# SheepYang666/VINA-SLAM

Measured on AMD Instinct MI355X. Metric: scans/sec (downsample+kNN+LM solve), 64-line LiDAR, 1/2/4/8 MI355X; ATE vs CPU, higher is better.
Workload: dtype f64

## Files before the change

### vina-slam_amd/csrc/insert.hip

```cpp
#include <cstring>
#include <vector>
#include "vg_map.h"

namespace vg {

template <bool kPre>
__global__ void __launch_bounds__(256) k_ins_prep(int n_arg, const int* __restrict__ nd, const float* __restrict__ ox, const float* __restrict__ oy,
                           const float* __restrict__ oz, const float* __restrict__ oi, MP mp, DState* __restrict__ st, int slot,
                           DevMap m, double* __restrict__ pw, uint32_t* __restrict__ hslot,
                           const PushArg* __restrict__ pa, const double* __restrict__ pin, const double* __restrict__ xsrc,
                           int var_identity, int* __restrict__ dsf, unsigned long long* __restrict__ gran, int ngran,
                           const int* __restrict__ ph_in) {
  const int n = nd ? *nd : n_arg;
  {
    const int g = blockIdx.x * blockDim.x + threadIdx.x;
    if (gran && g < ngran) gran[g] = 0ull;
  }
  if (!kPre && pa && blockIdx.x == 0) push_state_block(st, *pa);
  if (ph_in && blockIdx.x == 0 && threadIdx.x < 6) st->ph[threadIdx.x] = ph_in[threadIdx.x];
  const double* xc = kPre ? xsrc : st->xc;
  M3 R, rot_var, tsl_var;
  for (int r = 0; r < 3; r++)
    for (int c = 0; c < 3; c++) {
      R(r, c) = xc[r * 3 + c];
// ... 216 lines not shown
    const int upto = last ? ntile : b;
    int a0 = 0, a1 = 0, a2 = 0, t0 = 0, t1 = 0, t2 = 0;
    for (int k = lane; k < upto; k += 64) {
      u64 g;
      for (long it = 0;; it++) {
        g = __hip_atomic_load(&gran[k], __ATOMIC_RELAXED, __HIP_MEMORY_SCOPE_AGENT);
        if (g >> 63) break;
        __builtin_amdgcn_s_sleep(1);
        if (it > (1l << 24)) {
          atomicOr(&m.counters[kCntErr], 64);
          g = 1ull << 63;
          break;
        }
      }
      const int c0 = (int)(g & kF), c1 = (int)((g >> 21) & kF), c2 = (int)((g >> 42) & kF);
      if (k < b) {
        a0 += c0;
        a1 += c1;
        a2 += c2;
      }
      t0 += c0;
      t1 += c1;
      t2 += c2;
    }
    for (int o = 32; o > 0; o >>= 1) {
      a0 += __shfl_down(a0, o, 64);
      a1 += __shfl_down(a1, o, 64);
      a2 += __shfl_down(a2, o, 64);
      t0 += __shfl_down(t0, o, 64);
      t1 += __shfl_down(t1, o, 64);
      t2 += __shfl_down(t2, o, 64);
    }
    if (lane == 0) {
      s_off[0] = a0;
      s_off[1] = a1;
      s_off[2] = a2;
      s_tot[0] = t0;
      s_tot[1] = t1;
      s_tot[2] = t2;
    }
  }
  __syncthreads();
  const int base = m.counters[kCntNew], sbase = m.counters[kCntSlideBase];
#pragma unroll
  for (int k = 0; k < 4; k++) {
    const int i = i0 + k;
    const int cd = code[k];
    const u64 rk = r;
    r += pack3(cd);
    if (i >= n || !(cd & 1)) continue;
    const uint32_t s = hslot[i];
    int rt;
    if (cd & 2) {
      rt = base + s_off[1] + (int)((rk >> 21) & kF);
      if (rt >= m.cap_nodes) {
        atomicOr(&m.counters[kCntErr], 4);
        continue;
      }
      const uint64_t key = m.hkey[s];
      double c[3];
      const int64_t kk[3] = {unpack_axis(key, 42), unpack_axis(key, 21), unpack_axis(key, 0)};
      for (int j = 0; j < 3; j++) c[j] = (0.5 + kk[j]) * mp.vs;
      init_node(m.hdr[rt], c, (float)(mp.vs / 4.0), 0, -1);
      dbox_root(m.dbox + (size_t)rt * 6);
      m.hval[s] = rt;
    } else {
      rt = m.hval[s];
      m.hdr[rt].isexist = 1;
    }
    if (cd & 4) {
      m.in_slide[rt] = 1;
      m.slide[sbase + s_off[2] + (int)((rk >> 42) & kF)] = rt;
    }
    m.hfirst[s] = 0x7f7f7f7f;
  }
  if (b == ntile - 1 && tid == 0) {
    m.counters[kCntNodes] = min(base + s_tot[1], m.cap_nodes);
    m.counters[kCntRoots] = s_tot[1];
    m.counters[kCntTouched] = s_tot[0];
    m.counters[kCntSlide] = sbase + s_tot[2];
  }
}

__device__ __forceinline__ bool ins_skip(const DevMap& m, int thread_num) {
  return g_touched(m) < thread_num || m.counters[kCntMisc] != 0;
}

template <bool kCount>
__global__ void __launch_bounds__(256) k_ins_descend(int n_arg, const int* __restrict__ nd, int thread_num, const double* __restrict__ pw, DevMap m,
                                                     const uint32_t* __restrict__ hslot, int* __restrict__ leaf,
                                                     int* __restrict__ reqlist, int* __restrict__ seg_key) {
  const int n = nd ? *nd : n_arg;
  if (ins_skip(m, thread_num)) return;
  for (int base = blockIdx.x * blockDim.x; base < n; base += gridDim.x * blockDim.x) {
    const int i = base + threadIdx.x;
    int node = -1;
    bool first = false;
    if (i < n) {
      const uint32_t hs = hslot[i];
      node = hs != 0xffffffffu ? m.hval[hs] : -1;
    }
    if (node >= 0) {
      V3 w = v3(pw[3 * i], pw[3 * i + 1], pw[3 * i + 2]);
      for (int d = 0; d < 8; d++) {
        const NodeHdr& h = m.hdr[node];
        if (h.octo == 0) break;
        int o = octant(w, h.center);
        int c = h.child[o];
        if (c < 0) {
          if (atomicCAS(&m.cfirst[(size_t)node * 8 + o], 0x7f7f7f7f, -5) == 0x7f7f7f7f) {
            first = true;
            if (atomicExch(&m.nscr[(size_t)node * 4 + 1], -7) != -7) {
              int pos = atomicAdd(&m.counters[kCntCreate], 1);
              reqlist[pos] = node;
            }
          }
          if (kCount) atomicAdd(&m.creq_cnt[(size_t)node * 8 + o], 1);
          node = -2 - (node * 8 + o);
          break;
        }
        node = c;
      }
      if (kCount && node >= 0) first = atomicAdd(&m.leaf_cnt[node], 1) == 0;
    }
    if (i < n) leaf[i] = node;
    if (kCount) {
      const int s = wave_append(&m.counters[kCntSeg], first ? 1 : 0);
      if (first) seg_key[s] = node;
    }
  }
}

__global__ void __launch_bounds__(256) k_ins_resolve(int n_arg, const int* __restrict__ nd, int thread_num, const double* __restrict__ pw, DevMap m,
                                                     int* __restrict__ leaf, int* __restrict__ seg_leaf) {
  const int n = nd ? *nd : n_arg;
  if (ins_skip(m, thread_num)) return;
  for (int base = blockIdx.x * blockDim.x; base < n; base += gridDim.x * blockDim.x) {
    const int i = base + threadIdx.x;
    int node = i < n ? leaf[i] : -1;
    if (node < -1) {
      const int code = -2 - node;
      node = m.hdr[code >> 3].child[code & 7];
      leaf[i] = node;
    }
    const bool first = node >= 0 && atomicAdd(&m.leaf_cnt[node], 1) == 0;
    const int s = wave_append(&m.counters[kCntSeg], first ? 1 : 0);
    if (first) {
      seg_leaf[s] = node;
      m.leaf_seg[node] = s;
    }
  }
}

__global__ void __launch_bounds__(1024) k_seg_offsets(int thread_num, DevMap m, const int* __restrict__ seg_leaf,
                                                      int* __restrict__ seg_off) {
  __shared__ int s_w[17];
  if (ins_skip(m, thread_num)) return;
  const int ns = m.counters[kCntSeg];
  const int per = (ns + (int)blockDim.x - 1) / (int)blockDim.x;
  const int s0 = threadIdx.x * per, s1 = min(ns, s0 + per);
  constexpr int kPer = 32;
  int total;
  if (per <= kPer) {
    int lf[kPer], c[kPer];
#pragma unroll
    for (int k = 0; k < kPer; k++) lf[k] = s0 + k < s1 ? seg_leaf[s0 + k] : -1;
    int cnt = 0;
#pragma unroll
    for (int k = 0; k < kPer; k++) {
      c[k] = lf[k] >= 0 ? m.leaf_cnt[lf[k]] : 0;
      cnt += c[k];
    }
    int pos = block_excl_scan(cnt, s_w, &total);
#pragma unroll
    for (int k = 0; k < kPer; k++)
      if (lf[k] >= 0) {
        seg_off[s0 + k] = pos;
        pos += c[k];
        m.leaf_cnt[lf[k]] = 0;
      }
  } else {
    int cnt = 0;
// ... 298 lines not shown
                                                        int cap, const int* __restrict__ seg_key,
                                                        int2* __restrict__ seg_ol) {
  __shared__ int sp[kInsAllocCap];
  __shared__ int s_w[17];
  if (blockIdx.x == 0) {
    ins_alloc_block(thread_num, m, reqlist, cap, sp, s_w);
    return;
  }
  if (g_touched(m) < thread_num) return;
  const int ns = m.counters[kCntSeg];
  for (int base = ((int)blockIdx.x - 1) * (int)blockDim.x; base < ns; base += ((int)gridDim.x - 1) * (int)blockDim.x) {
    const int s = base + threadIdx.x;
    int* c = s < ns ? seg_counter(m, seg_key[s]) : nullptr;
    const int len = c ? *c : 0;
    const int off = wave_append(&m.counters[kCntSegCur], len);
    if (c) {
      seg_ol[s] = make_int2(off, len);
      *c = off;
    }
  }
}

__global__ void __launch_bounds__(256) k_ins_scatter_cur(int n_arg, const int* __restrict__ nd, int thread_num, DevMap m,
                                                         const int* __restrict__ leaf, int* __restrict__ order) {
  const int n = nd ? *nd : n_arg;
  if (ins_skip(m, thread_num)) return;
  for (int i = blockIdx.x * blockDim.x + threadIdx.x; i < n; i += gridDim.x * blockDim.x) {
    const int l = leaf[i];
    if (l == -1) continue;
    order[atomicAdd(seg_counter(m, l), 1)] = i;
  }
}

static int insert_tail(vg_ctx* ctx, const MP& mp, int slot, int n, int thread_num, const int* nd = nullptr) {
  DevMap& m = ctx->map;
  Work& w = ctx->wk;
  hipStream_t s = ctx->stream;
  const int g = grid_for(n);
  const int gseg = (n + kPushWaves - 1) / kPushWaves < 2048 ? (n + kPushWaves - 1) / kPushWaves : 2048;
  int* seg_leaf = w.list1;
  int* seg_off = reinterpret_cast<int*>(w.v0);
  int* order = reinterpret_cast<int*>(w.k0);
  int* order2 = reinterpret_cast<int*>(w.k1);
  const bool cur = ctx->ins_count;
  if (cur) {
    k_ins_scatter_cur<<<g * (kBlock / kSpreadBlock), kSpreadBlock, 0, s>>>(n, nd, thread_num, m, w.leaf, order);
  } else {
    k_ins_resolve<<<g * (kBlock / kSpreadBlock), kSpreadBlock, 0, s>>>(n, nd, thread_num, w.pw, m, w.leaf, seg_leaf);
    k_seg_offsets<<<1, 1024, 0, s>>>(thread_num, m, seg_leaf, seg_off);
    k_ins_scatter<<<g * (kBlock / kSpreadBlock), kSpreadBlock, 0, s>>>(n, nd, thread_num, m, w.leaf, seg_off, order);
  }
  RcBeginArg rb;
  memset(&rb, 0, sizeof(rb));
  const bool has_rb = ctx->rc_begin_wa != nullptr;
  if (has_rb) {
    rb.wa = *ctx->rc_begin_wa;
    rb.st = ctx->st;
    rb.wpn = m.wpn;
    rb.win = (WinD*)ctx->ba.xs;
    rb.nper = (int*)((char*)ctx->ba.xs + sizeof(WinD));
    rb.slot_of = rb.nper + 32;
    rb.rc = w.rc;
    ctx->rc_begin_wa = nullptr;
    ctx->rc_begun = true;
  }
  auto push = cur ? (ctx->push_pipe ? k_push_window<true, true> : k_push_window<true, false>)
                  : (ctx->push_pipe ? k_push_window<false, true> : k_push_window<false, false>);
  push<<<gseg + (has_rb ? 1 : 0), 64 * kPushWaves, 0, s>>>(seg_leaf, seg_off, order, order2, mp, slot, m, w.pw, thread_num,
                                                            rb, has_rb ? 1 : 0);
  VG_HIP(hipGetLastError());
  return VG_OK;
}

int map_insert(vg_ctx* ctx, const MP& mp, int slot, int n, int epoch, int thread_num, const PushArg* push,
               const InsPre* pre, const int* nd) {
  DevMap& m = ctx->map;
  Work& w = ctx->wk;
  hipStream_t s = ctx->stream;
  if (n <= 0) {
    if (push) VG_TRY(state_push(ctx, push->ord, push->new_imu, push->rec));
    return VG_OK;
  }
  const int g = nd ? grid_for(n, kBlock, 2048) : grid_for(n);
  if (pre)
    k_ins_prep<true><<<g, kBlock, 0, s>>>(n, nullptr, nullptr, nullptr, nullptr, nullptr, mp, ctx->st, slot, m, w.pw,
                                          w.u0,
                                          nullptr, pre->pnt, pre->pose, pre->var_identity, nullptr, w.gran, w.ngran,
                                          nullptr);
  else {
    HostIn* hin = ctx->h_in + ctx->in_sel;
    HostIn* din = ctx->d_in + ctx->in_sel;
    if (push) hin->push = *push;
    k_ins_prep<false><<<g, kBlock, 0, s>>>(n, nd, ctx->ds.ox, ctx->ds.oy, ctx->ds.oz, ctx->ds.oi, mp, ctx->st, slot, m,
                                           w.pw,
                                           w.u0, push ? &din->push : nullptr, nullptr, nullptr, 0,
                                           nd ? ctx->ds.hflags : nullptr, w.gran, w.ngran,
                                           ctx->in_ph ? din->ph : nullptr);
  }
  const int ntile = (n + kRootTile - 1) / kRootTile;
  (void)epoch;
  if (ctx->roots_lb && ntile <= w.ngran) {
    k_ins_roots_lb<<<ntile, kBlock, 0, s>>>(n, nd, ntile, w.u0, mp, m, w.gran);
  } else {
    k_ins_flags<<<ntile, kBlock, 0, s>>>(n, nd, w.u0, m, w.v1, (int*)w.ac_cnt);
    k_ins_roots_alloc<<<ntile, kBlock, 0, s>>>(n, nd, ntile, w.u0, w.v1, (const int*)w.ac_cnt, mp, m);
  }
  if (sharded(ctx)) {
    VG_TRY(shard_allreduce(ctx, m.counters + kCntTouched, m.counters + kCntGTouched, 1, 1, 1));
  }
  const int ins_cap = (ctx->dbg_ins_cap >= 0 && ctx->dbg_ins_cap < kInsAllocCap) ? ctx->dbg_ins_cap : kInsAllocCap;
  if (ctx->ins_count) {
    k_ins_descend<true><<<g * (kBlock / kSpreadBlock), kSpreadBlock, 0, s>>>(n, nd, thread_num, w.pw, m, w.u0, w.leaf,
                                                                             w.list2, w.list1);
    k_ins_alloc_seg<<<1 + kSegAllocBlocks, 1024, 0, s>>>(thread_num, m, w.list2, ins_cap, w.list1,
                                                         reinterpret_cast<int2*>(w.v0));
  } else {
    k_ins_descend<false><<<g * (kBlock / kSpreadBlock), kSpreadBlock, 0, s>>>(n, nd, thread_num, w.pw, m, w.u0, w.leaf,
                                                                              w.list2, nullptr);
    k_ins_alloc<<<1, 1024, 0, s>>>(thread_num, m, w.list2, ins_cap);
  }
  return insert_tail(ctx, mp, slot, n, thread_num, nd);
}

int map_insert_replay(vg_ctx* ctx, const MP& mp, int slot, int n, int thread_num) {
  DevMap& m = ctx->map;
  hipStream_t s = ctx->stream;
  VG_TRY(read_counters(ctx));
  const int np = ctx->h_pinned[kCntCreate];
  VG_HIP(hipMemsetAsync(m.counters + kCntMisc, 0, sizeof(int), s));
  if (!ctx->ins_count) VG_HIP(hipMemsetAsync(m.counters + kCntSeg, 0, sizeof(int), s));
  int created = 0;
  VG_TRY(alloc_children(ctx, ctx->wk.list2, np, nullptr, 0, false, &created));
  return insert_tail(ctx, mp, slot, n, thread_num);
}

int map_insert_segments(vg_ctx* ctx, int* key, int* len, int cap, int* info) {
  DevMap& m = ctx->map;
  Work& w = ctx->wk;
  hipStream_t s = ctx->stream;
  int hc[kCntN];
  VG_HIP(hipMemcpyAsync(hc, m.counters, sizeof(hc), hipMemcpyDeviceToHost, s));
  VG_HIP(hipStreamSynchronize(s));
  const int ns = hc[kCntSeg];
  info[0] = ns;
  info[1] = hc[kCntTouched];
  info[2] = hc[kCntCreate];
  info[3] = hc[kCntMisc];
  const int k = ns < cap ? ns : cap;
  if (k <= 0) return VG_OK;
  std::vector<int> off((size_t)2 * k + 2);
  VG_HIP(hipMemcpyAsync(key, w.list1, (size_t)k * sizeof(int), hipMemcpyDeviceToHost, s));
  VG_HIP(hipMemcpyAsync(off.data(), w.v0, (ctx->ins_count ? (size_t)2 * k : (size_t)k + 1) * sizeof(int),
                        hipMemcpyDeviceToHost, s));
  VG_HIP(hipStreamSynchronize(s));
  for (int q = 0; q < k; q++) len[q] = ctx->ins_count ? off[2 * q + 1] : off[q + 1] - off[q];
  return VG_OK;
}

}
```

### vina-slam_amd/csrc/map.hip

```cpp
#include <hipcub/hipcub.hpp>
#include "vg_map.h"

namespace vg {

int map_alloc(vg_ctx* ctx) {
  DevMap& m = ctx->map;
  const int W = ctx->cfg.win_size;
  m.W = W;
  m.cap_nodes = ctx->cap.max_nodes;
  m.cap_fix = ctx->cap.max_fix_points;
  m.hash_mask = (1 << ctx->cap.hash_log2) - 1;
  m.cap_wp = ctx->cap.max_points_per_scan;
  const size_t cn = m.cap_nodes, hs = (size_t)m.hash_mask + 1, cw = (size_t)m.cap_wp;
  auto ok = [&](void* p) { return p != nullptr; };
  bool good = true;
  good &= ok(m.hdr = ctx->arena.take<NodeHdr>(cn));
  good &= ok(m.pl = ctx->arena.take<PlaneRec>(cn));
  good &= ok(m.pcr_add = ctx->arena.take<Clu>(cn));
  good &= ok(m.pcr_fix = ctx->arena.take<Clu>(cn));
  good &= ok(m.cov_add = ctx->arena.take<double>(cn * kCovN));
  good &= ok(m.eig = ctx->arena.take<double>(cn * 12));
  good &= ok(m.jour = ctx->arena.take<double>(cn));
  good &= ok(m.dbox = ctx->arena.take<double>(cn * 6));
  good &= ok(m.pcrs = ctx->arena.take<Clu>(cn * W));
  good &= ok(m.nscr = ctx->arena.take<int>(cn * 4));
  good &= ok(m.pend = ctx->arena.take<unsigned long long>(cn));
  good &= ok(m.cfirst = ctx->arena.take<int>(cn * 8));
  good &= ok(m.hkey = ctx->arena.take<uint64_t>(hs));
  good &= ok(m.hval = ctx->arena.take<int>(hs));
  good &= ok(m.hfirst = ctx->arena.take<int>(hs));
  good &= ok(m.slide = ctx->arena.take<int>(cn));
  good &= ok(m.in_slide = ctx->arena.take<uint8_t>(cn));
  good &= ok(m.leaf_cnt = ctx->arena.take<int>(cn));
  good &= ok(m.leaf_seg = ctx->arena.take<int>(cn));
  good &= ok(m.creq_cnt = ctx->arena.take<int>(cn * 8));
  good &= ok(m.fix_pnt = ctx->arena.take<double>((size_t)m.cap_fix * 3));
  good &= ok(m.fix_var = ctx->arena.take<double>((size_t)m.cap_fix * 9));
  good &= ok(m.wp_pnt = ctx->arena.take<double>(cw * W * 3));
  good &= ok(m.wp_var = ctx->arena.take<double>(cw * W * 9));
  good &= ok(m.wp_leaf = ctx->arena.take<int>(cw * W));
  good &= ok(m.wp_int = ctx->arena.take<float>(cw * W));
  m.ord_stride = (int)(cw * (size_t)(ctx->cfg.max_layer + 1));
  good &= ok(m.wp_ord = ctx->arena.take<int>((size_t)m.ord_stride * W));
  good &= ok(m.lseg = ctx->arena.take<uint64_t>(cn * W));
  good &= ok(m.slot_epoch = ctx->arena.take<int>(kMaxWin));
  good &= ok(m.arena = ctx->arena.take<int>(kMaxWin));
  good &= ok(ctx->d_cmap = ctx->arena.take<float4>((cw + 2) / 3));
  good &= ok(ctx->d_cmap_n = ctx->arena.take<int>(4));
  good &= ok(m.counters = ctx->arena.take<int>(kCntN));
  good &= ok(m.stamp = ctx->arena.take<int>(cn));
  good &= ok(m.wpn = ctx->arena.take<int>(kMaxWin));
  Work& w = ctx->wk;
  w.cap = (int)(cw * (W + 1));
  good &= ok(w.k0 = ctx->arena.take<uint64_t>(w.cap));
  good &= ok(w.k1 = ctx->arena.take<uint64_t>(w.cap));
  good &= ok(w.v0 = ctx->arena.take<uint32_t>(w.cap));
  good &= ok(w.v1 = ctx->arena.take<uint32_t>(w.cap));
  good &= ok(w.u0 = ctx->arena.take<uint32_t>(w.cap));
  good &= ok(w.u1 = ctx->arena.take<uint32_t>(w.cap));
  good &= ok(w.ac_cnt = ctx->arena.take<uint32_t>(cn));
  good &= ok(w.ac_off = ctx->arena.take<uint32_t>(cn));
  good &= ok(w.cand = ctx->arena.take<int>(cn));
  good &= ok(w.list0 = ctx->arena.take<int>(cn));
  good &= ok(w.list1 = ctx->arena.take<int>(cn));
  good &= ok(w.list2 = ctx->arena.take<int>(cn));
  good &= ok(w.leaf = ctx->arena.take<int>(cw));
  good &= ok(w.pw = ctx->arena.take<double>(cw * 3));
  good &= ok(w.iekf_cache = ctx->arena.take<int>(cw));
  good &= ok(w.pk_leaf = ctx->arena.take<int>(cw));
  good &= ok(w.rc = ctx->arena.take<int>(128));
  good &= ok(w.cand_bits = ctx->arena.take<uint32_t>(ctx->cap.max_nodes / 32 + 1));
  good &= ok(w.plan = ctx->arena.take<int>(cn * 8));
  w.ngran = (int)(cw / 1024 + 64);
  good &= ok(w.gran = ctx->arena.take<unsigned long long>(w.ngran));
  good &= ok(w.sub_odd = ctx->arena.take<int>(cn));
  good &= ok(w.info_odd = ctx->arena.take<int>(w.cap));
  good &= ok(w.ev_odd = ctx->arena.take<uint64_t>(w.cap));
  w.nparts = 1024;
  good &= ok(w.partials = ctx->arena.take<double>((size_t)w.nparts * 40));
  if (!good) {
    ctx->err = "arena exhausted (map)";
    return VG_E_CAPACITY;
  }
  size_t b1 = 0, b2 = 0;
  VG_HIP(hipcub::DeviceRadixSort::SortKeys(nullptr, b1, w.k0, w.k1, w.cap, 0, 64, ctx->stream));
  VG_HIP(hipcub::DeviceScan::ExclusiveSum(nullptr, b2, w.v0, w.v1, w.cap, ctx->stream));
  w.tmp_bytes = (b1 > b2 ? b1 : b2) + 256;
  w.tmp = ctx->arena.take<char>(w.tmp_bytes);
  w.tmp2 = ctx->arena.take<char>(w.tmp_bytes);
  if (!w.tmp || !w.tmp2) {
    ctx->err = "arena exhausted (sort workspace)";
    return VG_E_CAPACITY;
  }
  return VG_OK;
}

int map_reset(vg_ctx* ctx) {
  DevMap& m = ctx->map;
  hipStream_t s = ctx->stream;
  int used = m.cap_nodes;
  if (ctx->pool_zeroed) {
    VG_HIP(hipMemcpyAsync(ctx->h_pinned, m.counters, kCntN * sizeof(int), hipMemcpyDeviceToHost, s));
    VG_HIP(hipStreamSynchronize(s));
    used = ctx->h_pinned[kCntNodes] < m.cap_nodes ? ctx->h_pinned[kCntNodes] : m.cap_nodes;
  }
  if (used > 0) {
    const size_t u = (size_t)used;
    VG_HIP(hipMemsetAsync(m.pl, 0, u * sizeof(PlaneRec), s));
    VG_HIP(hipMemsetAsync(m.pcr_add, 0, u * sizeof(Clu), s));
    VG_HIP(hipMemsetAsync(m.pcr_fix, 0, u * sizeof(Clu), s));
    VG_HIP(hipMemsetAsync(m.cov_add, 0, u * kCovN * sizeof(double), s));
    VG_HIP(hipMemsetAsync(m.eig, 0, u * 12 * sizeof(double), s));
    VG_HIP(hipMemsetAsync(m.jour, 0, u * sizeof(double), s));
    VG_HIP(hipMemsetAsync(m.pcrs, 0, u * m.W * sizeof(Clu), s));
    VG_HIP(hipMemsetAsync(m.lseg, 0, u * m.W * sizeof(uint64_t), s));
  }
  ctx->pool_zeroed = true;
  const size_t hs = (size_t)m.hash_mask + 1;
  VG_HIP(hipMemsetAsync(m.hkey, 0xff, hs * sizeof(uint64_t), s));
  VG_HIP(hipMemsetAsync(m.hval, 0xff, hs * sizeof(int), s));
  VG_HIP(hipMemsetAsync(m.hfirst, 0x7f, hs * sizeof(int), s));
  VG_HIP(hipMemsetAsync(m.counters, 0, kCntN * sizeof(int), s));
  VG_HIP(hipMemsetAsync(m.stamp, 0, (size_t)m.cap_nodes * sizeof(int), s));
  VG_HIP(hipMemsetAsync(m.wpn, 0, kMaxWin * sizeof(int), s));
  VG_HIP(hipMemsetAsync(m.slot_epoch, 0, kMaxWin * sizeof(int), s));
  VG_HIP(hipMemsetAsync(m.arena, 0, kMaxWin * sizeof(int), s));
  VG_HIP(hipMemsetAsync(ctx->wk.cand_bits, 0, (ctx->cap.max_nodes / 32 + 1) * sizeof(uint32_t), s));
  VG_HIP(hipMemsetAsync(m.in_slide, 0, m.cap_nodes, s));
  VG_HIP(hipMemsetAsync(m.leaf_cnt, 0, (size_t)m.cap_nodes * sizeof(int), s));
  VG_HIP(hipMemsetAsync(m.cfirst, 0x7f, (size_t)m.cap_nodes * 8 * sizeof(int), s));
  VG_HIP(hipMemsetAsync(m.creq_cnt, 0, (size_t)m.cap_nodes * 8 * sizeof(int), s));
  VG_HIP(hipMemsetAsync(m.nscr, 0xff, (size_t)m.cap_nodes * 4 * sizeof(int), s));
  VG_HIP(hipStreamSynchronize(s));
  return ds_reset(ctx);
}

int read_counters(vg_ctx* ctx) {
  VG_HIP(hipMemcpyAsync(ctx->h_pinned, ctx->map.counters, kCntN * sizeof(int), hipMemcpyDeviceToHost,
                        ctx->stream));
  VG_HIP(stream_wait(ctx));
  if (ctx->h_pinned[kCntErr]) {
    int e = ctx->h_pinned[kCntErr];
    ctx->err = std::string("device map error flags=") + std::to_string(e) +
               ((e & 4) ? " (node pool full)" : "") + ((e & 8) ? " (point_fix arena full)" : "") +
               ((e & 1) ? " (voxel key out of packed range)" : "") + ((e & 2) ? " (root hash full)" : "") +
               ((e & 16) ? " (subdivision event buffer full)" : "");
    return (e & 1) ? VG_E_RANGE : VG_E_CAPACITY;
  }
  return VG_OK;
}

static int excl_scan(vg_ctx* ctx, const uint32_t* in, uint32_t* out, int n) {
  size_t tb = ctx->wk.tmp_bytes;
  if (n <= 0) return VG_OK;
  VG_HIP(hipcub::DeviceScan::ExclusiveSum(ctx->wk.tmp, tb, in, out, n, ctx->stream));
  return VG_OK;
}
static int bits_for(long v) {
  int b = 1;
  while ((1L << b) <= v) b++;
  return b;
}

int sort_ids(vg_ctx* ctx, int* a, int n, int** result) {
  *result = a;
  if (n <= 1) return VG_OK;
  Work& w = ctx->wk;
  hipcub::DoubleBuffer<uint32_t> db(reinterpret_cast<uint32_t*>(a), w.u1);
  size_t tb = w.tmp_bytes;
  VG_HIP(hipcub::DeviceRadixSort::SortKeys(w.tmp, tb, db, n, 0, bits_for(ctx->map.cap_nodes), ctx->stream));
  *result = reinterpret_cast<int*>(db.Current());
  return VG_OK;
}
int sort_ids_inplace(vg_ctx* ctx, int* a, int n) {
  int* r = a;
  VG_TRY(sort_ids(ctx, a, n, &r));
  if (r != a) VG_HIP(hipMemcpyAsync(a, r, (size_t)n * sizeof(int), hipMemcpyDeviceToDevice, ctx->stream));
  return VG_OK;
}

__global__ void __launch_bounds__(256) k_child_count(int np, const int* __restrict__ parents, DevMap m, uint32_t* __restrict__ cnt) {
  for (int q = blockIdx.x * blockDim.x + threadIdx.x; q < np; q += gridDim.x * blockDim.x) {
    int p = parents[q];
    int c = 0;
    for (int o = 0; o < 8; o++) c += (m.cfirst[(size_t)p * 8 + o] == -5) ? 1 : 0;
    cnt[q] = (uint32_t)c;
  }
}

__global__ void __launch_bounds__(256) k_child_alloc(int np, const int* __restrict__ parents, const uint32_t* __restrict__ off, DevMap m,
                              int* __restrict__ next, int next_base) {
  const int base = m.counters[kCntNodes];
  for (int q = blockIdx.x * blockDim.x + threadIdx.x; q < np; q += gridDim.x * blockDim.x)
    alloc_parent(m, parents[q], base + (int)off[q], next, next_base + (int)off[q]);
}

__global__ void __launch_bounds__(256) k_add_counter(int* counters, int idx, const uint32_t* __restrict__ flag,
                              const uint32_t* __restrict__ rank, int n) {
  if (threadIdx.x == 0 && blockIdx.x == 0 && n > 0) counters[idx] += (int)(rank[n - 1] + flag[n - 1]);
}

int alloc_children(vg_ctx* ctx, int* plist, int np, int* next, int next_base, bool sorted, int* n_created) {
  Work& w = ctx->wk;
  hipStream_t s = ctx->stream;
  *n_created = 0;
  if (np <= 0) return VG_OK;
  if (!sorted) VG_TRY(sort_ids_inplace(ctx, plist, np));
  VG_TRY(read_counters(ctx));
  int first = ctx->h_pinned[kCntNodes];
  k_child_count<<<grid_for(np), kBlock, 0, s>>>(np, plist, ctx->map, w.ac_cnt);
  VG_TRY(excl_scan(ctx, w.ac_cnt, w.ac_off, np));
  k_child_alloc<<<grid_for(np), kBlock, 0, s>>>(np, plist, w.ac_off, ctx->map, next, next_base);
  k_add_counter<<<1, 64, 0, s>>>(ctx->map.counters, kCntNodes, w.ac_cnt, w.ac_off, np);
  VG_HIP(hipGetLastError());
// ... 7 lines not shown
```

### vina-slam_amd/csrc/vg_internal.h

```cpp
#pragma once
#include <hip/hip_runtime.h>
#include <chrono>
#include <functional>
#include <mutex>
#include <cstdint>
#include <string>
#include <thread>
#include <vector>
#include "../../include/vina_gpu.h"
#include "vg_la.h"
#include "vg_scratch.h"

#define VG_HIP(call)                                                                    \
  do {                                                                                  \
    hipError_t e_ = (call);                                                             \
    if (e_ != hipSuccess) {                                                             \
      ctx->err = std::string(#call) + ": " + hipGetErrorString(e_);                    \
      return VG_E_HIP;                                                                  \
    }                                                                                   \
  } while (0)

#define VG_TRY(expr)            \
  do {                          \
    int r_ = (expr);            \
// ... 441 lines not shown
  bool flag_force = false;
  vg::HostIn* h_in = nullptr;
  vg::HostIn* d_in = nullptr;
  int in_sel = 0;
  bool in_ph = false;
  hipGraphExec_t g_scan[vg::kMaxWin] = {};
  bool scan_graph = true;
  int ba_seq0_pre = 0;
  bool ba_no_defer = false;
  unsigned rc_flag_ctr = 0, pre_flag_ctr = 0;
  bool pool_zeroed = false;
  bool ins_ev_pending = false;
  bool use_graphs = true;
  bool overlap_iekf = true;
  int pub_flags = 0;
  vg::DevBuf<vg_plane_marker> d_mk;
  vg::DevBuf<int> d_mk_cnt;
  int mk_cap = 1 << 16;
  bool mk_fresh = false;
  bool mk_keep = false;
  float4* d_cmap = nullptr;
  int* d_cmap_n = nullptr;
  bool ds_early = true;
  bool ds_after_iekf = true;
  bool spec_tail = true;
  std::string err;
  vg::Arena arena;
  float *d_x = nullptr, *d_y = nullptr, *d_z = nullptr, *d_i = nullptr, *d_t = nullptr;
  const float *cur_x = nullptr, *cur_y = nullptr, *cur_z = nullptr, *cur_i = nullptr;
  int cur_n = -1;
  vg::DownsampleBufs ds;
  vg::KdMap kd;
  vg::DevMap map;
  vg::Work wk;
  vg::BaBufs ba;
  vg::DState* st = nullptr;
  vg::Shard shard;
  vg::Pub* h_pub = nullptr;
  vg::Pub* d_pub = nullptr;
  double* h_stage = nullptr;
  double* d_deskew = nullptr;
  int pub_seq = 0;
  int wait_spin_us = 0, wait_sleep_us = 0;
  int plane_tag = 0;
  int* h_pinned = nullptr;
  struct InSlot {
    char* h = nullptr;
    float* d = nullptr;
    hipEvent_t up = nullptr;
    hipEvent_t done = nullptr;
    bool live = false;
  } in_slot[2];
  size_t in_cap = 0;
  void* copy_pool = nullptr;
  int in_next = 0;
  hipEvent_t in_ev = nullptr;

  bool mapping = true;
  vg_ctx* view_of = nullptr;
  int views = 0;
  vg::DevMap own_map;
  void* fleet = nullptr;
  vg::ScoreBufs score;
  vg::RayBufs ray;
  vg::InfoBufs info;
  vg::OccBufs occ;
  vg::ClrBufs clr;
  vg::NavBufs nav;
  vg::FrontierBufs fr;
  vg::ChangeLayer* change = nullptr;
  std::mutex change_mu;
  vg::PlaceIndex* places = nullptr;
  std::mutex places_mu;
  vg_stats stats;
  void* host = nullptr;
  bool prof_on = false;
  int prof_every = 0;
  long prof_runs = 0;
  int rc_total = 0, rc_thread_num = 0;
  bool prof_stages = false;
  bool ins_count = true;
  bool push_pipe = false;
  bool roots_lb = true;
  bool ba_graph2 = true;
  bool margi_batch = true;
  bool margi_fused = true;
  bool iekf_prefetch = true;
  bool ba_structural = true;
  bool ba_resid_hess = true;
  bool ba_init_hess = true;
  bool rc_init_finish = true;
  bool rc_finish_in_init = false;
  bool rc_begin_fold = true;
  const vg::WinArg* rc_begin_wa = nullptr;
  bool rc_begun = false;
  bool ba_fuse_ctl = true;
  bool ba_graph = true;
  bool flag_sync = true;
  unsigned* d_sync = nullptr;
  bool sync_tail_armed = false;
  unsigned sync_tail_value = 0, sync_iekf_value = 0;
  bool dev_prop = false;
  bool rc_fused = true;
  bool prof_clock = false;
  hipEvent_t prof_ev[8][2] = {};
  hipEvent_t sync_ev = nullptr;
  hipEvent_t iekf_ev[16][2] = {};
  int iekf_ring_n = 0, iekf_ring_base = 0;
  hipEvent_t solve_ev[10][2] = {};
  int dbg_apply_cap = -1;
  int dbg_ins_cap = -1;
  int dbg_fac_max = -1;
  int dbg_capture = 0;
  double* dbg_cap_buf = nullptr;
  int dbg_cap_n = 0;
  bool prof_pending[16] = {};
  double prof_ms[16] = {};
  int prof_n[16] = {};
};

namespace vg {
constexpr int kTrajRow = 13;
constexpr int kPathRow = 14;
constexpr size_t kStageBytes = 1 << 17;
constexpr size_t kStageDeskewOff = 8192;
constexpr int kDeskewBuf = 4096;
inline void wait_pause(const vg_ctx* c, long spin, std::chrono::steady_clock::time_point t0);
inline int pub_wait(vg_ctx* c, const int* flag, int seq, const char* what, hipStream_t producer = nullptr) {
  hipStream_t st = producer ? producer : c->stream;
  const auto t0 = std::chrono::steady_clock::now();
  for (long spin = 0; __atomic_load_n(flag, __ATOMIC_ACQUIRE) < seq; spin++) {
    wait_pause(c, spin, t0);
    if ((spin & 4095) == 4095) {
      const hipError_t e = hipStreamQuery(st);
      if (e != hipSuccess && e != hipErrorNotReady) {
        c->err = std::string(what) + ": " + hipGetErrorString(e);
        return VG_E_HIP;
      }
      if (e == hipSuccess && __atomic_load_n(flag, __ATOMIC_ACQUIRE) < seq) {
        c->err = std::string(what) + ": stream drained without publishing";
        return VG_E_HIP;
      }
    }
  }
  return VG_OK;
}
enum { kProfDownsample = 0, kProfIekfKernel = 1, kProfInsert = 2, kProfRecut = 3, kProfBA = 4, kProfMargi = 5,
       kProfIekf = 6, kProfBaSolve = 7, kProfN = 8,
       kHostPropagate = 8, kHostDownsample = 9, kHostIekf = 10, kHostPush = 11, kHostInsert = 12, kHostRecut = 13,
       kHostBA = 14, kHostMargi = 15, kProfAll = 16 };
struct HostTimer {
  vg_ctx* c;
  int id;
  std::chrono::steady_clock::time_point t0;
  HostTimer(vg_ctx* ctx, int i) : c(ctx), id(i), t0(std::chrono::steady_clock::now()) {}
  ~HostTimer() {
    if (!c->prof_on) return;
    c->prof_ms[id] += std::chrono::duration<double, std::milli>(std::chrono::steady_clock::now() - t0).count();
    c->prof_n[id] += 1;
  }
};
inline void prof_begin(vg_ctx* c, int id, hipStream_t s = nullptr) {
  if (c->prof_stages) (void)hipEventRecord(c->prof_ev[id][0], s ? s : c->stream);
}
inline void prof_end(vg_ctx* c, int id, hipStream_t s = nullptr) {
  if (c->prof_stages) {
// ... 338 lines not shown
```

### vina-slam_amd/csrc/vina_gpu.cpp

```cpp
#include <algorithm>
#include <atomic>
#include <condition_variable>
#include <csignal>
#include <cstdio>
#include <execinfo.h>
#include <unistd.h>
#include <cstdlib>
#include <mutex>
#include <cstring>
#include <new>
#include <vector>
#include "vg_internal.h"

using namespace vg;

namespace {
struct CopyPool {
  struct Job {
    char* dst;
    const char* src;
    size_t bytes;
  };
  std::vector<std::thread> th;
  std::mutex mu;
// ... 868 lines not shown
          if (e > k.h_t0[slot]) {
            t += e - k.h_t0[slot];
            nl++;
          }
        }
    }
    if (stage == vg::kProfAll) {
      t = 0;
      nl = 0;
      const int nb = vg::iekf_grid(ctx) < vg::kClkBlocks ? vg::iekf_grid(ctx) : vg::kClkBlocks;
      for (int sc = s0; sc <= s1; sc++)
        for (int it = 0; it < 4; it++) {
          const int slot = (sc * 4 + it) & (vg::kClkRing - 1);
          if (!k.exec[slot]) continue;
          unsigned long long e = 0;
          for (int b = 0; b < nb; b++) e = k.tend[slot][b] > e ? k.tend[slot][b] : e;
          if (e > k.t0[slot]) {
            t += e - k.t0[slot];
            nl++;
          }
        }
    }
    *total_ms = khz > 0 ? (double)t / (double)khz : 0.0;
    *count = (int)nl;
    return VG_OK;
  }
  *total_ms = ctx->prof_ms[stage];
  *count = ctx->prof_n[stage];
  return VG_OK;
}

}

extern "C" int vgx_debug(vg_ctx* ctx, int key, int value) {
  if (!ctx) return VG_E_ARG;
  if (key == 2) {
    ctx->use_graphs = value != 0;
    return VG_OK;
  }
  if (key == 1) {
    ctx->dbg_apply_cap = value;
    return VG_OK;
  }
  if (key == 3) {
    ctx->dbg_ins_cap = value;
    return VG_OK;
  }
  if (key == 4) {
    ctx->dbg_fac_max = value;
    return VG_OK;
  }
  if (key == 12) {
    if (!ctx->shard.d_seq) return VG_E_STATE;
    unsigned s = 0;
    VG_HIP(hipMemcpy(&s, ctx->shard.d_seq, sizeof(s), hipMemcpyDeviceToHost));
    s += (unsigned)value;
    VG_HIP(hipMemcpy(ctx->shard.d_seq, &s, sizeof(s), hipMemcpyHostToDevice));
    return VG_OK;
  }
  if (key == 24) {
    ctx->margi_batch = value != 0;
    return VG_OK;
  }
  if (key == 23) {
    ctx->iekf_prefetch = value != 0;
    return VG_OK;
  }
  if (key == 21) {
    ctx->margi_fused = value != 0;
    return VG_OK;
  }
  if (key == 19) {
    ctx->ba_fuse_ctl = value != 0;
    return VG_OK;
  }
  if (key == 17) {
    ctx->ba_graph2 = value != 0;
    return VG_OK;
  }
  if (key == 38) {
    ctx->ins_count = value != 0;
    return VG_OK;
  }
  if (key == 39) {
    ctx->push_pipe = value != 0;
    return VG_OK;
  }
  if (key == 16) {
    ctx->roots_lb = value != 0;
    return VG_OK;
  }
  if (key == 15) {
    ctx->ba_graph = value != 0;
    return VG_OK;
  }
  if (key == 37) {
    ctx->ds_after_iekf = value != 0;
    return VG_OK;
  }
  if (key == 35) {
    ctx->ba_init_hess = value != 0;
    return VG_OK;
  }
  if (key == 34) {
    ctx->ba_resid_hess = value != 0;
    return VG_OK;
  }
  if (key == 33) {
    ctx->rc_begin_fold = value != 0;
    return VG_OK;
  }
  if (key == 32) {
    ctx->rc_init_finish = value != 0;
    return VG_OK;
  }
  if (key == 31) {
    ctx->ba_structural = value != 0;
    return VG_OK;
  }
  if (key == 30) {
    ctx->shard_force = value != 0;
    return VG_OK;
  }
  if (key == 14) {
    ctx->flag_sync = value != 0;
    ctx->flag_force = value == 2;
    return VG_OK;
  }
  if (key == 27) {
    ctx->scan_graph = value != 0;
    return VG_OK;
  }
  if (key == 26) {
    ctx->lm_defer = value != 0;
    return VG_OK;
  }
  if (key == 13) {
    ctx->dev_prop = value != 0;
    return VG_OK;
  }
  if (key == 11) {
    ctx->rc_fused = value != 0;
    return VG_OK;
  }
  if (key == 7) {
    ctx->overlap_iekf = value != 0;
    return VG_OK;
  }
  if (key == 9) {
    ctx->ds_early = value != 0;
    return VG_OK;
  }
  if (key == 8) {
    ctx->spec_tail = value != 0;
    return VG_OK;
  }
  if (key == 5) {
    if (!ctx->dbg_cap_buf)
      VG_HIP(hipMalloc((void**)&ctx->dbg_cap_buf, (size_t)(4096 + 32 * 931) * sizeof(double)));
    ctx->dbg_capture = value ? 1 : 0;
    ctx->dbg_cap_n = 0;
    return VG_OK;
  }
  return VG_E_ARG;
}

// ... 139 lines not shown
```

Measured before the change: 1997.

## Fuse insert prep and root allocation into one decoupled-lookback kernel

Adds a single kernel that transforms points to world frame, inserts voxel keys into the root hash, and allocates new root nodes. It uses a two-phase inter-block flag protocol on the granule array: first a barrier waiting for all earlier tiles' hash inserts, then a decoupled lookback scan for the allocation offsets. This replaces the separate prep and roots kernels with one launch, and the hfirst reset and granule clearing move into the descend kernel. It relies on forward progress of earlier blocks with spin-waits, and it enlarges the granule buffer so that finer 256-point tiles fit.

```diff
diff --git a/vina-slam_amd/csrc/insert.hip b/vina-slam_amd/csrc/insert.hip
--- a/vina-slam_amd/csrc/insert.hip
+++ b/vina-slam_amd/csrc/insert.hip
@@ -322,22 +322,205 @@
   }
 }
 
+constexpr int kPrepTile = 256;
+__global__ void __launch_bounds__(256) k_ins_prep_roots(int n_arg, const int* __restrict__ nd, const float* __restrict__ ox,
+                                                        const float* __restrict__ oy, const float* __restrict__ oz,
+                                                        const float* __restrict__ oi, MP mp, DState* __restrict__ st, int slot,
+                                                        DevMap m, double* __restrict__ pw, uint32_t* __restrict__ hslot,
+                                                        const PushArg* __restrict__ pa, int* __restrict__ dsf,
+                                                        unsigned long long* __restrict__ gran, const int* __restrict__ ph_in) {
+  const int n = nd ? *nd : n_arg;
+  __shared__ u64 s_w[4];
+  __shared__ int s_off[3], s_tot[3], s_base[2];
+  const int tid = threadIdx.x, lane = tid & 63, b = blockIdx.x;
+  const int ntile = max(1, (n + kPrepTile - 1) / kPrepTile);
+  if (b >= ntile) return;
+  if (tid == 0) {
+    s_base[0] = m.counters[kCntNodes];
+    s_base[1] = m.counters[kCntSlide];
+  }
+  if (pa && b == 0) push_state_block(st, *pa);
+  if (ph_in && b == 0 && tid < 6) st->ph[tid] = ph_in[tid];
+  if (b == 0 && tid == 0) {
+    m.counters[kCntNew] = s_base[0];
+    m.counters[kCntSlideBase] = s_base[1];
+    m.counters[kCntCreate] = 0;
+    m.counters[kCntSeg] = 0;
+    m.counters[kCntSegCur] = 0;
+    m.counters[kCntMisc] = 0;
+    m.counters[kCntPlaneUpd] = 0;
+    m.counters[kCntFixFull] = 0;
+    m.counters[kCntNds] = n;
+    m.wpn[slot] = n;
+    m.slot_epoch[slot] += 1;
+    m.arena[slot] = m.cap_wp;
+    if (dsf && dsf[0]) {
+      atomicOr(&m.counters[kCntErr], 1);
+      dsf[0] = 0;
+    }
+  }
+  const int i = b * kPrepTile + tid;
+  uint32_t hs = 0xffffffffu;
+  uint64_t key = 0;
+  if (i < n) {
+    const double* xc = st->xc;
+    M3 R, rot_var, tsl_var;
+    for (int r = 0; r < 3; r++)
+      for (int c = 0; c < 3; c++) {
+        R(r, c) = xc[r * 3 + c];
+        rot_var(r, c) = xc[kXS + r * 15 + c];
+        tsl_var(r, c) = xc[kXS + (3 + r) * 15 + 3 + c];
+      }
+    const V3 p = ld_v3(xc + 9);
+    V3 pnt;
+    M3 var;
+    var_init_pt(mp, ox[i], oy[i], oz[i], pnt, var);
+    const M3 vw = world_var(R, var, pnt, rot_var, tsl_var);
+    const V3 w = rigid(R, pnt, p);
+    const size_t base = (size_t)slot * m.cap_wp + i;
+    for (int j = 0; j < 3; j++) m.wp_pnt[base * 3 + j] = pnt[j];
+    for (int j = 0; j < 9; j++) m.wp_var[base * 9 + j] = vw[j];
+    m.wp_leaf[base] = -1;
+    m.wp_int[base] = oi ? oi[i] : 0.f;
+    for (int j = 0; j < 3; j++) pw[(size_t)i * 3 + j] = w[j];
+    if (!pack_key(w, mp.vs, key)) {
+      atomicOr(&m.counters[kCntErr], 1);
+    } else if (owns(m, key)) {
+      bool fresh;
+      const int s = hash_insert(m.hkey, m.hash_mask, key, fresh);
+      if (s < 0) {
+        atomicOr(&m.counters[kCntErr], 2);
+      } else {
+        hs = (uint32_t)s;
+        atomicMin(&m.hfirst[s], i);
+      }
+    }
+    hslot[i] = hs;
+  }
+  asm volatile("s_waitcnt vmcnt(0)" ::: "memory");
+  __syncthreads();
+  if (tid == 0) __hip_atomic_store(&gran[b], 1ull << 62, __ATOMIC_RELAXED, __HIP_MEMORY_SCOPE_AGENT);
+  if (tid < 64) {
+    for (int k = lane; k < b; k += 64)
+      for (long it = 0;; it++) {
+        if (__hip_atomic_load(&gran[k], __ATOMIC_RELAXED, __HIP_MEMORY_SCOPE_AGENT) >> 62) break;
+        __builtin_amdgcn_s_sleep(1);
+        if (it > (1l << 24)) {
+          atomicOr(&m.counters[kCntErr], 64);
+          break;
+        }
+      }
+  }
+  __syncthreads();
+  int cd = 0, rt = -1;
+  if (hs != 0xffffffffu && __hip_atomic_load(&m.hfirst[hs], __ATOMIC_RELAXED, __HIP_MEMORY_SCOPE_AGENT) == i) {
+    rt = m.hval[hs];
+    cd = rt < 0 ? 7 : (m.in_slide[rt] ? 1 : 5);
+  }
+  u64 tot;
+  const u64 rk = block_excl_scan3(pack3(cd), s_w, &tot);
+  constexpr u64 kF = (1ull << 21) - 1;
+  if (tid == 0) __hip_atomic_store(&gran[b], tot | (1ull << 63), __ATOMIC_RELAXED, __HIP_MEMORY_SCOPE_AGENT);
+  if (tid < 64) {
+    const bool last = b == ntile - 1;
+    const int upto = last ? ntile : b;
+    int a0 = 0, a1 = 0, a2 = 0, t0 = 0, t1 = 0, t2 = 0;
+    for (int k = lane; k < upto; k += 64) {
+      u64 g;
+      for (long it = 0;; it++) {
+        g = __hip_atomic_load(&gran[k], __ATOMIC_RELAXED, __HIP_MEMORY_SCOPE_AGENT);
+        if (g >> 63) break;
+        __builtin_amdgcn_s_sleep(1);
+        if (it > (1l << 24)) {
+          atomicOr(&m.counters[kCntErr], 64);
+          g = 1ull << 63;
+          break;
+        }
+      }
+      const int c0 = (int)(g & kF), c1 = (int)((g >> 21) & kF), c2 = (int)((g >> 42) & 0xfffffu);
+      if (k < b) {
+        a0 += c0;
+        a1 += c1;
+        a2 += c2;
+      }
+      t0 += c0;
+      t1 += c1;
+      t2 += c2;
+    }
+    for (int o = 32; o > 0; o >>= 1) {
+      a0 += __shfl_down(a0, o, 64);
+      a1 += __shfl_down(a1, o, 64);
+      a2 += __shfl_down(a2, o, 64);
+      t0 += __shfl_down(t0, o, 64);
+      t1 += __shfl_down(t1, o, 64);
+      t2 += __shfl_down(t2, o, 64);
+    }
+    if (lane == 0) {
+      s_off[0] = a0;
+      s_off[1] = a1;
+      s_off[2] = a2;
+      s_tot[0] = t0;
+      s_tot[1] = t1;
+      s_tot[2] = t2;
+    }
+  }
+  __syncthreads();
+  const int nbase = s_base[0], sbase = s_base[1];
+  if (cd & 1) {
+    bool ok = true;
+    if (cd & 2) {
+      rt = nbase + s_off[1] + (int)((rk >> 21) & kF);
+      if (rt >= m.cap_nodes) {
+        atomicOr(&m.counters[kCntErr], 4);
+        ok = false;
+      } else {
+        double c[3];
+        const int64_t kk[3] = {unpack_axis(key, 42), unpack_axis(key, 21), unpack_axis(key, 0)};
+        for (int j = 0; j < 3; j++) c[j] = (0.5 + kk[j]) * mp.vs;
+        init_node(m.hdr[rt], c, (float)(mp.vs / 4.0), 0, -1);
+        dbox_root(m.dbox + (size_t)rt * 6);
+        m.hval[hs] = rt;
+      }
+    } else {
+      m.hdr[rt].isexist = 1;
+    }
+    if (ok && (cd & 4)) {
+      m.in_slide[rt] = 1;
+      m.slide[sbase + s_off[2] + (int)((rk >> 42) & 0xfffffu)] = rt;
+    }
+  }
+  if (b == ntile - 1 && tid == 0) {
+    m.counters[kCntNodes] = min(nbase + s_tot[1], m.cap_nodes);
+    m.counters[kCntRoots] = s_tot[1];
+    m.counters[kCntTouched] = s_tot[0];
+    m.counters[kCntSlide] = sbase + s_tot[2];
+  }
+}
+
 __device__ __forceinline__ bool ins_skip(const DevMap& m, int thread_num) {
   return g_touched(m) < thread_num || m.counters[kCntMisc] != 0;
 }
 
-template <bool kCount>
+template <bool kCount, bool kFused = false>
 __global__ void __launch_bounds__(256) k_ins_descend(int n_arg, const int* __restrict__ nd, int thread_num, const double* __restrict__ pw, DevMap m,
                                                      const uint32_t* __restrict__ hslot, int* __restrict__ leaf,
-                                                     int* __restrict__ reqlist, int* __restrict__ seg_key) {
+                                                     int* __restrict__ reqlist, int* __restrict__ seg_key,
+                                                     unsigned long long* __restrict__ gran, int ntile) {
   const int n = nd ? *nd : n_arg;
-  if (ins_skip(m, thread_num)) return;
+  {
+    const int g = blockIdx.x * blockDim.x + threadIdx.x;
+    if (gran && g < ntile) gran[g] = 0ull;
+  }
+  const bool skip = ins_skip(m, thread_num);
+  if (!kFused && skip) return;
   for (int base = blockIdx.x * blockDim.x; base < n; base += gridDim.x * blockDim.x) {
     const int i = base + threadIdx.x;
     int node = -1;
     bool first = false;
     if (i < n) {
       const uint32_t hs = hslot[i];
+      if (kFused && hs != 0xffffffffu && m.hfirst[hs] == i) m.hfirst[hs] = 0x7f7f7f7f;
+      if (kFused && skip) continue;
       node = hs != 0xffffffffu ? m.hval[hs] : -1;
     }
     if (node >= 0) {
@@ -802,41 +985,55 @@
     return VG_OK;
   }
   const int g = nd ? grid_for(n, kBlock, 2048) : grid_for(n);
-  if (pre)
-    k_ins_prep<true><<<g, kBlock, 0, s>>>(n, nullptr, nullptr, nullptr, nullptr, nullptr, mp, ctx->st, slot, m, w.pw,
-                                          w.u0,
-                                          nullptr, pre->pnt, pre->pose, pre->var_identity, nullptr, w.gran, w.ngran,
-                                          nullptr);
-  else {
+  const int ntile_f = (n + kPrepTile - 1) / kPrepTile;
+  const bool fused = ctx->ins_onepass && !pre && ctx->ins_count && ctx->roots_lb && !sharded(ctx) && ntile_f <= w.ngran;
+  int ntile = (n + kRootTile - 1) / kRootTile;
+  (void)epoch;
+  if (fused) {
     HostIn* hin = ctx->h_in + ctx->in_sel;
     HostIn* din = ctx->d_in + ctx->in_sel;
     if (push) hin->push = *push;
-    k_ins_prep<false><<<g, kBlock, 0, s>>>(n, nd, ctx->ds.ox, ctx->ds.oy, ctx->ds.oz, ctx->ds.oi, mp, ctx->st, slot, m,
-                                           w.pw,
-                                           w.u0, push ? &din->push : nullptr, nullptr, nullptr, 0,
-                                           nd ? ctx->ds.hflags : nullptr, w.gran, w.ngran,
-                                           ctx->in_ph ? din->ph : nullptr);
-  }
-  const int ntile = (n + kRootTile - 1) / kRootTile;
-  (void)epoch;
-  if (ctx->roots_lb && ntile <= w.ngran) {
-    k_ins_roots_lb<<<ntile, kBlock, 0, s>>>(n, nd, ntile, w.u0, mp, m, w.gran);
+    ntile = ntile_f;
+    k_ins_prep_roots<<<ntile, kBlock, 0, s>>>(n, nd, ctx->ds.ox, ctx->ds.oy, ctx->ds.oz, ctx->ds.oi, mp, ctx->st,
+                                             slot, m, w.pw, w.u0, push ? &din->push : nullptr,
+                                             nd ? ctx->ds.hflags : nullptr, w.gran, ctx->in_ph ? din->ph : nullptr);
   } else {
-    k_ins_flags<<<ntile, kBlock, 0, s>>>(n, nd, w.u0, m, w.v1, (int*)w.ac_cnt);
-    k_ins_roots_alloc<<<ntile, kBlock, 0, s>>>(n, nd, ntile, w.u0, w.v1, (const int*)w.ac_cnt, mp, m);
-  }
+    if (pre)
+      k_ins_prep<true><<<g, kBlock, 0, s>>>(n, nullptr, nullptr, nullptr, nullptr, nullptr, mp, ctx->st, slot, m, w.pw,
+                                            w.u0,
+                                            nullptr, pre->pnt, pre->pose, pre->var_identity, nullptr, w.gran, w.ngran,
+                                            nullptr);
+    else {
+      HostIn* hin = ctx->h_in + ctx->in_sel;
+      HostIn* din = ctx->d_in + ctx->in_sel;
+      if (push) hin->push = *push;
+      k_ins_prep<false><<<g, kBlock, 0, s>>>(n, nd, ctx->ds.ox, ctx->ds.oy, ctx->ds.oz, ctx->ds.oi, mp, ctx->st, slot, m,
+                                             w.pw,
+                                             w.u0, push ? &din->push : nullptr, nullptr, nullptr, 0,
+                                             nd ? ctx->ds.hflags : nullptr, w.gran, w.ngran,
+                                             ctx->in_ph ? din->ph : nullptr);
+    }
+    if (ctx->roots_lb && ntile <= w.ngran) {
+      k_ins_roots_lb<<<ntile, kBlock, 0, s>>>(n, nd, ntile, w.u0, mp, m, w.gran);
+    } else {
+      k_ins_flags<<<ntile, kBlock, 0, s>>>(n, nd, w.u0, m, w.v1, (int*)w.ac_cnt);
+      k_ins_roots_alloc<<<ntile, kBlock, 0, s>>>(n, nd, ntile, w.u0, w.v1, (const int*)w.ac_cnt, mp, m);
+    }
+  }
+  unsigned long long* gz = ctx->roots_lb && ntile <= w.ngran ? w.gran : nullptr;
   if (sharded(ctx)) {
     VG_TRY(shard_allreduce(ctx, m.counters + kCntTouched, m.counters + kCntGTouched, 1, 1, 1));
   }
   const int ins_cap = (ctx->dbg_ins_cap >= 0 && ctx->dbg_ins_cap < kInsAllocCap) ? ctx->dbg_ins_cap : kInsAllocCap;
   if (ctx->ins_count) {
-    k_ins_descend<true><<<g * (kBlock / kSpreadBlock), kSpreadBlock, 0, s>>>(n, nd, thread_num, w.pw, m, w.u0, w.leaf,
-                                                                             w.list2, w.list1);
+    auto descend = fused ? k_ins_descend<true, true> : k_ins_descend<true, false>;
+    descend<<<g * (kBlock / kSpreadBlock), kSpreadBlock, 0, s>>>(n, nd, thread_num, w.pw, m, w.u0, w.leaf, w.list2, w.list1,
+                                                                 gz, ntile);
     k_ins_alloc_seg<<<1 + kSegAllocBlocks, 1024, 0, s>>>(thread_num, m, w.list2, ins_cap, w.list1,
                                                          reinterpret_cast<int2*>(w.v0));
   } else {
     k_ins_descend<false><<<g * (kBlock / kSpreadBlock), kSpreadBlock, 0, s>>>(n, nd, thread_num, w.pw, m, w.u0, w.leaf,
-                                                                              w.list2, nullptr);
+                                                                              w.list2, nullptr, gz, ntile);
     k_ins_alloc<<<1, 1024, 0, s>>>(thread_num, m, w.list2, ins_cap);
   }
   return insert_tail(ctx, mp, slot, n, thread_num, nd);
diff --git a/vina-slam_amd/csrc/map.hip b/vina-slam_amd/csrc/map.hip
--- a/vina-slam_amd/csrc/map.hip
+++ b/vina-slam_amd/csrc/map.hip
@@ -71,7 +71,7 @@
   good &= ok(w.rc = ctx->arena.take<int>(128));
   good &= ok(w.cand_bits = ctx->arena.take<uint32_t>(ctx->cap.max_nodes / 32 + 1));
   good &= ok(w.plan = ctx->arena.take<int>(cn * 8));
-  w.ngran = (int)(cw / 1024 + 64);
+  w.ngran = (int)(cw / 256 + 64);
   good &= ok(w.gran = ctx->arena.take<unsigned long long>(w.ngran));
   good &= ok(w.sub_odd = ctx->arena.take<int>(cn));
   good &= ok(w.info_odd = ctx->arena.take<int>(w.cap));
@@ -130,6 +130,7 @@
   VG_HIP(hipMemsetAsync(m.leaf_cnt, 0, (size_t)m.cap_nodes * sizeof(int), s));
   VG_HIP(hipMemsetAsync(m.cfirst, 0x7f, (size_t)m.cap_nodes * 8 * sizeof(int), s));
   VG_HIP(hipMemsetAsync(m.creq_cnt, 0, (size_t)m.cap_nodes * 8 * sizeof(int), s));
+  VG_HIP(hipMemsetAsync(ctx->wk.gran, 0, (size_t)ctx->wk.ngran * sizeof(unsigned long long), s));
   VG_HIP(hipMemsetAsync(m.nscr, 0xff, (size_t)m.cap_nodes * 4 * sizeof(int), s));
   VG_HIP(hipStreamSynchronize(s));
   return ds_reset(ctx);
diff --git a/vina-slam_amd/csrc/vg_internal.h b/vina-slam_amd/csrc/vg_internal.h
--- a/vina-slam_amd/csrc/vg_internal.h
+++ b/vina-slam_amd/csrc/vg_internal.h
@@ -547,6 +547,7 @@
   bool ins_count = true;
   bool push_pipe = false;
   bool roots_lb = true;
+  bool ins_onepass = true;
   bool ba_graph2 = true;
   bool margi_batch = true;
   bool margi_fused = true;
diff --git a/vina-slam_amd/csrc/vina_gpu.cpp b/vina-slam_amd/csrc/vina_gpu.cpp
--- a/vina-slam_amd/csrc/vina_gpu.cpp
+++ b/vina-slam_amd/csrc/vina_gpu.cpp
@@ -974,6 +974,10 @@
     ctx->ins_count = value != 0;
     return VG_OK;
   }
+  if (key == 40) {
+    ctx->ins_onepass = value != 0;
+    return VG_OK;
+  }
   if (key == 39) {
     ctx->push_pipe = value != 0;
     return VG_OK;
```

New measurement: 2010, median of 6. Within noise of the previous version (+0.7%).
